# mhrice/RemFx

Measured on AMD Instinct MI355X. Metric: audio-seconds/sec fwd+bwd (whole job), higher is better.
Workload: dtype bf16 (fp32 accumulate); 1 GPU; Hybrid Demucs (cfg/model/demucs.yaml) train step, +exp=chorus_aug model=demucs; clips_per_gpu=64, global_batch=64, clip_samples=262144, parallelism=dp1, rccl_ranks=0, ranks=1, streams=4

## Files before the change

include/remfx_hip.h:

```cpp
#ifndef REMFX_HIP_H
#define REMFX_HIP_H

#include <stdint.h>

#ifdef __cplusplus
extern "C" {
#endif

#define RFX_ABI_VERSION 1

enum rfx_act {
  RFX_ACT_NONE = 0,
  RFX_ACT_RELU = 1,
  RFX_ACT_GELU = 2,
  RFX_ACT_TANH = 3,
  RFX_ACT_PRELU = 4,
  RFX_ACT_LEAKY = 5,
  RFX_ACT_SIGMOID = 6
};

typedef struct rfx_ktab_entry {
  int32_t off;
  int32_t da;
  int32_t db;
// ... 301 lines not shown
  int32_t N, IA, IB, OA, OB, SA;
  int32_t NTR, NCH, NTC, KS;
  int32_t da0, da_step;
  int32_t db0, db_step;
  int32_t wrapb;
  const void* apack;
  int32_t M, BM;
  int32_t mode;
  int32_t G, g_off, OAo, Co;
  const float* bias;
  const float* rowadd;
  rfx_cl_tensor out0, out1, aux0, res;
  void* cm_out;
  int64_t cm_ns, cm_cs, cm_as;
  int32_t cm_fold;
} rfx_cl_conv_desc;
int rfx_cl_conv(const rfx_cl_conv_desc* d, void* stream);
int rfx_cl_pack(const float* src, const int32_t* idx, int64_t n, void* dst, void* stream);
int rfx_cl_from_cm(const void* src, int32_t src_bf16, int64_t s_ns, int64_t s_cs, int64_t s_as, int32_t N, int32_t C, int32_t A,
                   int32_t B, const rfx_cl_tensor* dst, const rfx_cl_tensor* res, const rfx_cl_tensor* aux, int32_t mode, void* stream);
int rfx_cl_to_cm(const rfx_cl_tensor* src, int32_t N, int32_t C, int32_t A, int32_t B, void* dst, int32_t dst_bf16, int64_t d_ns,
                 int64_t d_cs, int64_t d_as, const void* aux16, void* stream);
int rfx_cl_im2col_s4(const float* src, int64_t s_ns, int64_t s_cs, int64_t s_as, int32_t N, int32_t Cs, int32_t IA, int32_t IB, int32_t OA,
                     int32_t OB, int32_t along_b, void* dst, void* stream);
int rfx_cl_im2col_fm(const float* src, const float* coef_a, const float* coef_b, int32_t N, int32_t F, int32_t bins, void* dst, void* stream);
int rfx_fm_cm_affine(const float* in, float* out, const float* coef_a, const float* coef_b, int32_t N, int32_t bins, int32_t F, int32_t to_fm,
                     void* stream);
int rfx_cl_dgelu(const void* g, const void* z, void* out, int64_t n, void* stream);
int rfx_cl_dglu(const void* g, const void* zab, void* out, int64_t npos, int32_t C, void* stream);

// ... 45 lines not shown
```

remfx_amd/_lib.py:

```python
import ctypes as C
import glob
import os
import subprocess

_HERE = os.path.dirname(os.path.abspath(__file__))
_ROOT = os.path.dirname(_HERE)
CSRC = os.path.join(_HERE, "csrc")
INCLUDE = os.path.join(_ROOT, "include")
LIBDIR = os.path.join(_HERE, "_C")
LIBPATH = os.environ.get("RFX_LIBPATH_DEV") or os.path.join(LIBDIR, "libremfx_hip.so")

HIPCC_FLAGS = ["--offload-arch=gfx950", "-O3", "-std=c++17", "-fPIC", "-ffp-contract=fast",
               "-I" + INCLUDE, "-I" + CSRC]


def sources():
    return sorted(glob.glob(os.path.join(CSRC, "*.hip")))


def _stale():
    if not os.path.exists(LIBPATH):
        return True
    t = os.path.getmtime(LIBPATH)
    deps = sources() + glob.glob(os.path.join(CSRC, "*.h")) + glob.glob(os.path.join(INCLUDE, "*.h"))
# ... 57 lines not shown
                                         "herm")] + \
               [(n, C.c_float) for n in ("scale", "eps", "alpha")] + [("accum", C.c_int32)]


class ClTensor(C.Structure):
    _fields_ = [("p", C.c_void_p), ("ns", C.c_int64), ("as_", C.c_int64), ("bs", C.c_int32), ("c0", C.c_int32)]


class ClConvDesc(C.Structure):
    _fields_ = [("inp", ClTensor)] + \
               [(n, C.c_int32) for n in ("N", "IA", "IB", "OA", "OB", "SA", "NTR", "NCH", "NTC", "KS", "da0", "da_step", "db0",
                                         "db_step", "wrapb")] + \
               [("apack", C.c_void_p)] + \
               [(n, C.c_int32) for n in ("M", "BM", "mode", "G", "g_off", "OAo", "Co")] + \
               [("bias", C.c_void_p), ("rowadd", C.c_void_p), ("out0", ClTensor), ("out1", ClTensor), ("aux0", ClTensor), ("res", ClTensor),
                ("cm_out", C.c_void_p), ("cm_ns", C.c_int64), ("cm_cs", C.c_int64), ("cm_as", C.c_int64), ("cm_fold", C.c_int32)]


class ClDconvDesc(C.Structure):
    _fields_ = [(n, C.c_void_p) for n in ("x", "gy", "y", "a", "hpre", "stats", "dz", "dh", "partial", "w1p", "w2p", "w2dp", "w1dp",
                                          "b1", "g1w", "g1b", "b2", "g2w", "g2b", "scale")] + \
               [(n, C.c_int32) for n in ("S", "C", "H", "dil", "grid", "x_or_gy_ok")] + [("eps", C.c_float), ("TPS", C.c_int32), ("tsum", C.c_void_p), ("sums", C.c_void_p), ("pg_dst", C.c_void_p * 5)]


class ClWgradDesc(C.Structure):
    _fields_ = [("p", ClTensor), ("q", ClTensor)] + \
               [(n, C.c_int32) for n in ("N", "OA", "IA", "B", "SA", "da0", "NTR", "NTC", "db0", "db_step", "M", "Cq", "CW", "RW", "WK",
                                         "S", "ahead", "bias", "PW")] + \
               [("ws", C.c_void_p)]


# ... 161 lines not shown
```

remfx_amd/clast.py:

```python
import ctypes as C
import os as _os

import numpy as np
import torch

from . import _lib, ops
from ._lib import ClConvDesc, ClTensor, ClWgradDesc, check

EPI = {"store": 0, "gelu": 1, "glu": 2, "dgelu": 3, "dglu": 4, "store_cm": 5}


def _stream():
    return C.c_void_p(ops.raw_stream())


def cl_tensor(t, c0=0):
    ct = ClTensor()
    if t is None:
        return ct
    if t.dtype != torch.bfloat16 or t.dim() != 4 or t.stride(3) != 1 or not t.is_cuda:
        raise ValueError(f"channels-last operand must be a 4-D bf16 GPU tensor with dense channels (got {t.dtype}, {tuple(t.shape)}, {t.stride()})")
    ct.p = t.data_ptr()
    ct.ns, ct.as_, ct.bs, ct.c0 = t.stride(0), t.stride(1), t.stride(2), c0
    return ct
# ... 104 lines not shown
        v = torch.from_numpy(form.idx).to(device)
        form._dev[key] = v
    return v


def pack(form, w):
    idx = _dev_index(form, w.device)
    wf = w if w.is_contiguous() else w.contiguous()
    out = torch.empty(idx.numel(), device=w.device, dtype=torch.bfloat16)
    check(_lib.lib().rfx_cl_pack(C.c_void_p(wf.data_ptr()), C.c_void_p(idx.data_ptr()), idx.numel(), C.c_void_p(out.data_ptr()),
                                 _stream()), "rfx_cl_pack")
    return out


def conv(form, apack, x, N, IA, IB, OA, mode, bias=None, out0=None, out1=None, aux0=None, res=None, OAo=0, x_c0=0, wrapb=False,
         rowadd=None, cm_out=None, cm_fold=False):
    d = ClConvDesc()
    d.inp = cl_tensor(x, x_c0)
    d.N, d.IA, d.IB, d.OA, d.OB, d.SA = N, IA, IB, OA, IB, form.SA
    d.NTR, d.NCH, d.NTC, d.KS = form.NTR, form.NCH, form.NTC, form.KS
    d.da0, d.da_step, d.db0, d.db_step = form.da0, form.da_step, form.db0, form.db_step
    d.wrapb = int(wrapb)
    d.apack = apack.data_ptr()
    d.M, d.BM, d.mode = form.M, form.BM, EPI[mode]
    d.G, d.g_off, d.OAo, d.Co = form.G, form.g_off, OAo, form.Co
    d.bias = bias.data_ptr() if bias is not None else None
    d.rowadd = rowadd.data_ptr() if rowadd is not None else None
    d.out0, d.out1, d.aux0, d.res = cl_tensor(out0), cl_tensor(out1), cl_tensor(aux0), cl_tensor(res)
    if cm_out is not None:
        if cm_out.dtype != torch.float32 or cm_out.stride(3) != 1:
            raise ValueError("store_cm: fp32 (N, C, rows, positions) with contiguous positions")
        d.cm_out, d.cm_ns, d.cm_cs, d.cm_as, d.cm_fold = cm_out.data_ptr(), cm_out.stride(0), cm_out.stride(1), cm_out.stride(2), int(cm_fold)
    check(_lib.lib().rfx_cl_conv(C.byref(d), _stream()), "rfx_cl_conv")


def form_conv_glu(Cout2, Cin, KA, KB):
    Ch = Cout2 // 2

    def widx(m, r, t, ch):
        oc = (m & 1) * Ch + (m >> 1)
        return ((oc * Cin + ch) * KA + r) * KB + t
    return ConvForm(Cout2, Cin, KA, KB, -(KA // 2), 1, -(KB // 2), 1, 1, widx)
# ... 284 lines not shown
```

remfx_amd/clchain.py:

```python
import ctypes as C

import torch

from . import _lib, clast, ops
from ._lib import check

_FORMS = {}
_BUILD = {
    "glu": clast.form_conv_glu, "dgrad": clast.form_conv_dgrad, "s4": clast.form_conv_s4, "s4d": clast.form_conv_s4_dgrad,
    "tr": clast.form_convtr_s4, "trd": clast.form_convtr_s4_dgrad, "w": clast.wform_conv, "ws4": clast.wform_conv_s4,
    "wtr": clast.wform_convtr_s4,
    "s4f": clast.form_conv_s4_fold, "s4fd": clast.form_conv_s4_fold_dgrad, "trf": clast.form_convtr_fold,
    "trfd": clast.form_convtr_fold_dgrad, "ws4f": clast.wform_conv_s4_fold, "wtrf": clast.wform_convtr_fold,
    "head": clast.form_head, "whead": clast.wform_head, "tail": clast.form_tail_tr, "taild": clast.form_tail_dgrad, "wtail": clast.wform_tail,
}


def _fold(t, k=4):
    N, A, L, Cc = t.shape
    return t.view(N, A, L // k, k * Cc)


def form(kind, *a):
    key = (kind,) + a
# ... 63 lines not shown
    return dw, db


def _scratch_bias(f, p):
    return torch.empty(f.M, device=p.device, dtype=torch.float32) if f.bias else None


def _as_ncab(x3, Bn, A):
    NA, Cc, T = x3.shape
    return x3.view(Bn, A, Cc, T).permute(0, 2, 1, 3)


class EncMidFn(torch.autograd.Function):

    @staticmethod
    def forward(ctx, d, rw_w, rw_b, cv_w, cv_b, emb_rows, Bn, y_cl, fold):
        d_is_cl = d.dim() == 4
        if d_is_cl:
            _, A, T, Cc = d.shape
            d_cl = d if d.is_contiguous() else d.contiguous()
        else:
            NA, Cc, T = d.shape
            A = NA // Bn
            d_cl = clast.from_cm(_as_ncab(d if d.is_contiguous() else d.contiguous(), Bn, A))
        C1 = cv_w.shape[0]
        A1, T1 = (A, T // 4) if fold else (A // 4, T)
        dev = d.device
        train = any(ctx.needs_input_grad)
        zab = clast.empty(Bn, A, T, 2 * Cc, dev) if train else None
        e = clast.empty(Bn, A, T, Cc, dev)
        fg = form("glu", 2 * Cc, Cc, 1, 1)
# ... 4 lines not shown
        if fold:
            fs = form("s4f", C1, Cc)
            clast.conv(fs, packed(fs, cv_w), _fold(e), Bn, 1, T1, 1, "gelu", bias=cv_b, out0=z1, out1=y1)
        else:
            fs = form("s4", C1, Cc)
            clast.conv(fs, packed(fs, cv_w), e, Bn, A, T, A1, "gelu", bias=cv_b, out0=z1, out1=y1)
        if y_cl:
            y_out = y1
        else:
            y_out = torch.empty((Bn * A1, C1, T1), device=dev, dtype=torch.float32)
            clast.to_cm(y1, out=_as_ncab(y_out, Bn, A1))
        if train:
            ctx.save_for_backward(d_cl, zab, e, z1, rw_w, cv_w)
            ctx.refs = (rw_b, cv_b)
            ctx.geom = (Bn, A, T, Cc, C1, A1, T1, emb_rows is not None, d_is_cl, y_cl, fold)
        return e, y_out

    @staticmethod
    def backward(ctx, g_e, g_y):
        d_cl, zab, e, z1, rw_w, cv_w = ctx.saved_tensors
        rw_b, cv_b = ctx.refs
        Bn, A, T, Cc, C1, A1, T1, has_emb, d_is_cl, y_cl, fold = ctx.geom
        dev = d_cl.device
        if y_cl:
            dz1 = clast.dgelu(g_y if g_y.is_contiguous() else g_y.contiguous(), z1)
        else:
            dz1 = clast.empty(Bn, A1, T1, C1, dev)
            clast.from_cm(_as_ncab(g_y if g_y.is_contiguous() else g_y.contiguous(), Bn, A1), out=dz1, aux=z1, mode="dgelu")
        g_e = (g_e if g_e.is_contiguous() else g_e.contiguous()) if g_e is not None else None
        if fold:
            dcw, dcb = _wgrad(form("ws4f", C1, Cc), dz1, _fold(e), Bn, 1, 1, T1, cv_w, cv_b)
            fd = form("s4fd", C1, Cc)
            v = clast.empty(Bn, A, T, Cc, dev)
            clast.conv(fd, packed(fd, cv_w), dz1, Bn, 1, T1, 1, "store", out0=_fold(v), res=_fold(g_e) if g_e is not None else None)
            dzab = clast.dglu(v, zab)
        else:
            dcw, dcb = _wgrad(form("ws4", C1, Cc), dz1, e, Bn, A1, A, T, cv_w, cv_b)
            fd = form("s4d", C1, Cc)
            dzab = clast.empty(Bn, A, T, 2 * Cc, dev)
            v = clast.empty(Bn, A, T, Cc, dev) if has_emb else None
            clast.conv(fd, packed(fd, cv_w), dz1, Bn, A1, T, A1 + 1, "dglu", out0=dzab, out1=v, aux0=zab, res=g_e, OAo=A)
        demb = None
        if has_emb:
            demb = torch.empty((A, Cc), device=dev, dtype=torch.float32)
            rowsum(v, A, Cc, demb)
        drw, drb = _wgrad(form("w", 2 * Cc, Cc, 1, 1), dzab, d_cl, Bn, A, A, T, rw_w, rw_b)
        fr = form("dgrad", 2 * Cc, Cc, 1, 1)
        dd_cl = clast.empty(Bn, A, T, Cc, dev)
        clast.conv(fr, packed(fr, rw_w), dzab, Bn, A, T, A, "store", out0=dd_cl)
        if d_is_cl:
            dd = dd_cl
        else:
            dd = torch.empty((Bn * A, Cc, T), device=dev, dtype=torch.float32)
            clast.to_cm(dd_cl, out=_as_ncab(dd, Bn, A))
        return dd, drw, drb, dcw, dcb, demb, None, None, None


class EncTailFn(torch.autograd.Function):

    @staticmethod
    def forward(ctx, d, rw_w, rw_b, Bn):
        d_is_cl = d.dim() == 4
        if d_is_cl:
            _, A, T, Cc = d.shape
            d_cl = d if d.is_contiguous() else d.contiguous()
        else:
            NA, Cc, T = d.shape
            A = NA // Bn
            d_cl = clast.from_cm(_as_ncab(d if d.is_contiguous() else d.contiguous(), Bn, A))
        dev = d.device
# ... 163 lines not shown
class HeadGeluFn(torch.autograd.Function):

    @staticmethod
    def forward(ctx, z):
        ctx.save_for_backward(z)
        return clast.from_cm(z, mode="gelu")

    @staticmethod
    def backward(ctx, g):
        (z,) = ctx.saved_tensors
        gz = torch.empty_like(z)
        clast.to_cm(g if g.is_contiguous() else g.contiguous(), out=gz, aux16=z)
        return gz


def head_gelu(z):
    if z.dtype != torch.bfloat16 or not z.is_contiguous():
        raise ValueError("head_gelu: contiguous bf16 (N, C, A, T)")
    return HeadGeluFn.apply(z)


def _w4(w):
    return w if w.dim() == 4 else w.unsqueeze(2)


def enc_mid(d, rewrite, conv_next, emb_rows, Bn, y_cl=False, fold=False):
    return EncMidFn.apply(d, _w4(rewrite.weight), rewrite.bias, _w4(conv_next.weight), conv_next.bias, emb_rows, Bn, y_cl, fold)


def enc_tail(d, rewrite, Bn):
    return EncTailFn.apply(d, _w4(rewrite.weight), rewrite.bias, Bn)


def freq_decoder(x, skips, layers, fold=False, tail=False):
    params = []
    for m in layers[:-1]:
        params += [_w4(m.rewrite.weight), m.rewrite.bias, _w4(m.conv_tr.weight), m.conv_tr.bias]
    params += [_w4(layers[-1].rewrite.weight), layers[-1].rewrite.bias]
    if tail:
        params += [_w4(layers[-1].conv_tr.weight), layers[-1].conv_tr.bias]
    return FreqDecoderFn.apply(x, len(skips), fold, tail, *skips, *params)


class HeadConvFn(torch.autograd.Function):

    @staticmethod
    def forward(ctx, x, w, b, along_b, coef=None):
        if coef is not None:
            Bn, T, IA, Cs = x.shape
            A = IA // 4
            x16 = clast.im2col_fm(x, coef[0], coef[1])
        else:
            Bn, Cs, IA, T = x.shape
            A, T = (IA, T // 4) if along_b else (IA // 4, T)
            x16 = clast.im2col_s4(x, A, T, along_b)
        Cc = w.shape[0]
        dev = x.device
        train = any(ctx.needs_input_grad[1:3])
        f = form("head", Cc, Cs)
        z = clast.empty(Bn, A, T, Cc, dev) if train else None
        y = clast.empty(Bn, A, T, Cc, dev)
        clast.conv(f, packed(f, w), x16, Bn, A, T, A, "gelu", bias=b, out0=z, out1=y)
        if train:
            ctx.save_for_backward(x16, z, w)
            ctx.refs = (b,)
        return y

    @staticmethod
    def backward(ctx, g):
        x16, z, w = ctx.saved_tensors
        (b,) = ctx.refs
        Bn, A, T, Cc = z.shape
        dz = clast.dgelu(g if g.is_contiguous() else g.contiguous(), z)
        dw, db = _wgrad(form("whead", Cc, w.shape[1]), dz, x16, Bn, A, A, T, w, b)
        return None, dw, db, None, None


def head_conv(x, conv, along_b=False):
    return HeadConvFn.apply(x, _w4(conv.weight), conv.bias, along_b)


def head_conv_fm(spec_fm, a, b, conv):
    return HeadConvFn.apply(spec_fm, _w4(conv.weight), conv.bias, False, (a, b))
```

remfx_amd/cldconv.py:

```python
import ctypes as C

import numpy as np
import torch

from . import _lib, clast, clchain, ops
from ._lib import ClDconvDesc, check

T = 256
import os as _os
GRID = 256
GRID_FWD = int(_os.environ.get("RFX_CLD_GRID_FWD", "256"))


class _Idx:

    def __init__(self, idx):
        self.idx = np.ascontiguousarray(idx.reshape(-1).astype(np.int32))
        self._dev = {}


_TABLES = {}


def tables(Cc, H):
# ... 64 lines not shown

def _p(t):
    return t.data_ptr() if t is not None else None


def _desc(Cc, H, dil, eps, S, b1, g1w, g1b, b2, g2w, g2b, scale):
    d = ClDconvDesc()
    d.S, d.C, d.H, d.dil, d.grid, d.eps = S, Cc, H, dil, GRID, eps
    d.b1, d.g1w, d.g1b, d.b2, d.g2w, d.g2b, d.scale = _p(b1), _p(g1w), _p(g1b), _p(b2), _p(g2w), _p(g2b), _p(scale)
    return d


class ClDconvLayerFn(torch.autograd.Function):

    @staticmethod
    def forward(ctx, x, w1, b1, g1w, g1b, w2, b2, g2w, g2b, scale, dil, eps):
        Bn, A, Tt, Cc = x.shape
        H = w1.shape[0]
        if Tt % T or not x.is_contiguous() or x.dtype != torch.bfloat16:
            raise ValueError("ClDconvLayerFn: dense (N, A, 256 k, C) bf16 input")
        tb = tables(Cc, H)
        TPS = Tt // T
        HP, S, dev = tb["HP"], Bn * A * TPS, x.device
        train = any(ctx.needs_input_grad)
        y = torch.empty_like(x)
        d = _desc(Cc, H, dil, eps, S, b1, g1w, g1b, b2, g2w, g2b, scale)
        d.TPS = TPS
        d.grid = GRID_FWD
        d.x, d.y = x.data_ptr(), y.data_ptr()
        d.w1p = clchain.packed(tb["w1p"], w1).data_ptr()
        d.w2p = clchain.packed(tb["w2p"], w2).data_ptr()
        a = hpre = stats = part = None
        if train or TPS > 1:
            stats = torch.empty((Bn * A, 4), device=dev, dtype=torch.float32)
            d.stats = stats.data_ptr()
        if TPS > 1:
            part = torch.empty((S, 2), device=dev, dtype=torch.float32)
            d.partial = part.data_ptr()
        if train:
            a = torch.empty((Bn, A, Tt, HP), device=dev, dtype=torch.bfloat16)
            hpre = torch.empty_like(a)
            d.a, d.hpre = a.data_ptr(), hpre.data_ptr()
        check(_lib.lib().rfx_cl_dconv_fwd(C.byref(d), C.c_void_p(ops.raw_stream())), "rfx_cl_dconv_fwd")
        if train:
            ctx.save_for_backward(x, a, hpre, stats, w1, b1, g1w, g1b, w2, b2, g2w, g2b, scale)
            ctx.cfg = (dil, eps)
        return y

    @staticmethod
    def backward(ctx, gy):
        x, a, hpre, stats, w1, b1, g1w, g1b, w2, b2, g2w, g2b, scale = ctx.saved_tensors
        dil, eps = ctx.cfg
        Bn, A, Tt, Cc = x.shape
        H = w1.shape[0]
        tb = tables(Cc, H)
        TPS = Tt // T
        HP, S, dev = tb["HP"], Bn * A * TPS, x.device
        passes = TPS > 1 or Cc != 48
        if not gy.is_contiguous():
            gy = gy.contiguous()
        dx = torch.empty_like(x)
        dz = torch.empty((Bn, A, Tt, 2 * Cc), device=dev, dtype=torch.bfloat16)
        dh = torch.empty((Bn, A, Tt, HP), device=dev, dtype=torch.bfloat16)
        npg = 5 * Cc + 2 * H
        partial = torch.empty((min(GRID, S), npg), device=dev, dtype=torch.float32)
        sink = ops.SINK
# ... 10 lines not shown
            tsum = torch.empty((S, 2), device=dev, dtype=torch.float32)
            sums = torch.empty((Bn * A, 4), device=dev, dtype=torch.float32)
            d.tsum, d.sums = tsum.data_ptr(), sums.data_ptr()
        else:
            d.w1dp = clchain.packed(tb["w1dp"], w1).data_ptr()
        if direct:
            for q, t in enumerate(tgt):
                d.pg_dst[q] = t[1].data_ptr()
        check(_lib.lib().rfx_cl_dconv_bwd(C.byref(d), C.c_void_p(pg.data_ptr() if pg is not None else None), C.c_void_p(ops.raw_stream())),
              "rfx_cl_dconv_bwd")
        if direct:
            for t in tgt:
                sink.wrote(t[0])
        if passes:
            fx = _dx_form(Cc, H, dil)
            clast.conv(fx, clchain.packed(fx, w1), dh, Bn, A, Tt, A, "store", out0=dx, res=gy)
        f1, f2 = _wforms(Cc, H, dil)
        dw2, db2 = clchain._wgrad(f2, dz, a, Bn, A, A, Tt, w2, b2)
        dw1, db1 = clchain._wgrad(f1, dh, x, Bn, A, A, Tt, w1, b1)
        if direct:
            dscale = dg2w = dg2b = dg1w = dg1b = None
        else:
            dscale, dg2w, dg2b = pg[:Cc], pg[Cc:3 * Cc], pg[3 * Cc:5 * Cc]
            dg1w, dg1b = pg[5 * Cc:5 * Cc + H], pg[5 * Cc + H:]
        return dx, dw1, db1, dg1w, dg1b, dw2, db2, dg2w, dg2b, dscale, None, None


def dconv_layer(x, conv1, gn1, conv2, gn2, scale, dil):
    return ClDconvLayerFn.apply(x, conv1.weight, conv1.bias, gn1.weight, gn1.bias, conv2.weight, conv2.bias, gn2.weight, gn2.bias,
                                scale, int(dil), float(gn1.eps))
```

remfx_amd/csrc/cl_conv.h:

```cpp
#pragma once
#include "cl_common.h"

#ifndef RFX_CLC_DBG_BUILD
#define RFX_CLC_DBG_BUILD 0
#endif

struct ClConvK {
  rfx_cl_conv_desc d;
  int32_t ptiles, chunk, MG, tpr;
  uint32_t in_bytes;
};

template <int RW, int NT, int WM, int NTC, int KS, int DA, int DB, bool HALO>
struct ClConvCfg {
  static constexpr int WN = 8 / WM, BM = 32 * RW * WM, MT = RW * WM;
  static constexpr int A_KB = NTC * KS * MT;
  static constexpr int PA = (A_KB + 3) / 4;
  static constexpr int SLOTS = HALO ? 272 : 256, CORE0 = HALO ? 16 : 0, PLANE = SLOTS * 32;
  static constexpr int PB = KS * (HALO ? 3 : 2);
  static constexpr int A_UNIT = A_KB * 1024, B_UNIT = KS * PLANE;
  static constexpr int RING = DA * A_UNIT + DB * B_UNIT;
  static constexpr int EPI_RS = 64 * RW + 8, EPI_RSY = 32 * RW + 8;
  static constexpr int EPI_WAVE = 32 * EPI_RS + 32 * EPI_RSY;
  static constexpr int BIAS_OFF = (RING > 8 * EPI_WAVE ? RING : 8 * EPI_WAVE);
// ... 355 lines not shown
        cl_unpack8(raw, v);
        if (mode == RFX_CL_GELU || mode == RFX_CL_DGELU) {
          if (has0) cl_bst(rs0, off0, raw);
          float w[8];
          if (has_aux) cl_unpack8(cl_bld(rsx, (uint32_t)(((int64_t)orow * d.aux0.as + (int64_t)bp * d.aux0.bs + ch) * 2)), w);
          float o[8];
          if (mode == RFX_CL_GELU) {
#pragma unroll
            for (int e = 0; e < 8; ++e) o[e] = rfx_gelu(v[e]) + (has_aux ? w[e] : 0.f);
          } else {
#pragma unroll
            for (int e = 0; e < 8; ++e) o[e] = v[e] * rfx_gelu_grad(w[e]);
          }
          cl_bst(rs1, (uint32_t)(((int64_t)orow * d.out1.as + (int64_t)bp * d.out1.bs + ch) * 2), cl_pack8(o));
        } else {
          const uint32_t ax = (uint32_t)(((int64_t)orow * d.aux0.as + (int64_t)bp * d.aux0.bs + ch) * 2);
          const int half = d.aux0.bs >> 1;
          float a[8], b[8], ga[8], gb[8];
          if (has1) cl_bst(rs1, (uint32_t)(((int64_t)orow * d.out1.as + (int64_t)bp * d.out1.bs + ch) * 2), raw);
          cl_unpack8(cl_bld(rsx, ax), a);
          cl_unpack8(cl_bld(rsx, ax + half * 2), b);
#pragma unroll
          for (int e = 0; e < 8; ++e) {
            const float s = rfx_sigmoid(b[e]);
            ga[e] = v[e] * s;
            gb[e] = v[e] * a[e] * s * (1.f - s);
          }
          cl_bst(rs0, off0, cl_pack8(ga));
          cl_bst(rs0, off0 + half * 2, cl_pack8(gb));
        }
      }
    }
    __builtin_amdgcn_wave_barrier();
    CL_LGKM0();
  }
}

template <int MODE, int RW, int NT, int WM, int NTC, int KS, int DA, int DB, bool HALO>
static int cl_conv_launch(const ClConvK& k, dim3 grid, hipStream_t s) {
  using Cfg = ClConvCfg<RW, NT, WM, NTC, KS, DA, DB, HALO>;
  static bool attr_done = false;
  if (!attr_done) {
    if (hipFuncSetAttribute(reinterpret_cast<const void*>(&cl_conv_kernel<MODE, RW, NT, WM, NTC, KS, DA, DB, HALO>),
                            hipFuncAttributeMaxDynamicSharedMemorySize, Cfg::LDS) != hipSuccess)
// ... 41 lines not shown
```

remfx_amd/csrc/cl_conv.hip:

```cpp
#include "cl_conv.h"

static bool cl_fits32(const rfx_cl_tensor& t, int rows, int IB) {
  if (!t.p) return true;
  return ((int64_t)rows * t.as + (int64_t)IB * t.bs) * 2 < 0x7fffffffLL && t.bs % 8 == 0 && t.c0 % 8 == 0;
}

extern "C" int rfx_cl_conv(const rfx_cl_conv_desc* dp, void* stream) {
  if (!dp || !dp->in.p || !dp->apack) return -1;
  const rfx_cl_conv_desc& d = *dp;
  if (d.N <= 0 || d.OA <= 0 || d.OB <= 0 || d.OB % 256 || d.OB != d.IB || d.M <= 0 || d.NTR <= 0 || d.NTR > 16 || d.NCH <= 0) return -1;
  if (d.in.bs % 8 || d.in.c0 % 8 || (d.NCH * 16 * d.KS + d.in.c0) > d.in.bs) return -1;
  const bool cm = d.mode == RFX_CL_STORE_CM;
  if (d.G < 1 || d.G > 4 || (d.G > 1 && ((!cm && d.Co % 8) || d.Co * d.G != d.M))) return -1;
  if (d.mode < 0 || d.mode > RFX_CL_STORE_CM) return -1;
  if (cm && (!d.cm_out || d.Co <= 0 || d.M % d.Co || d.BM != 32)) return -1;
  if (d.mode == RFX_CL_GLU && (d.M % 16 || !d.out1.p || d.G != 1)) return -1;
  if ((d.mode == RFX_CL_STORE || d.mode == RFX_CL_DGLU) && !d.out0.p) return -1;
  if ((d.mode == RFX_CL_GELU || d.mode == RFX_CL_DGELU) && !d.out1.p) return -1;
  if ((d.mode == RFX_CL_DGELU || d.mode == RFX_CL_DGLU) && !d.aux0.p) return -1;
  if (d.M % 8 && !cm) return -1;
  const int orows = d.G > 1 ? d.OAo : d.OA;
  if (!cl_fits32(d.out0, orows, d.IB) || !cl_fits32(d.out1, orows, d.IB) || !cl_fits32(d.aux0, orows, d.IB) || !cl_fits32(d.res, orows, d.IB))
    return -1;
  const int64_t ext = ((int64_t)(d.IA - 1) * d.in.as + (int64_t)d.IB * d.in.bs - d.in.c0) * 2;
  if (ext <= 0 || ext >= 0x7fffffffLL) return -1;
  ClConvK k;
  k.d = d;
  k.tpr = d.OB / 256;
  k.ptiles = d.N * d.OA * k.tpr;
  k.chunk = (k.ptiles + 7) / 8;
  k.MG = (d.M + d.BM - 1) / d.BM;
  k.in_bytes = (uint32_t)ext;

  const dim3 grid((unsigned)(8 * k.chunk * k.MG));
// ... 28 lines not shown
```

remfx_amd/hdemucs.py:

```python
import math
import os

import torch
import torch.nn as nn
import torch.nn.functional as F

from . import clchain, cldconv, lstm, nnops, ops, stft

CL_TRUNK = os.environ.get("RFX_CL_TRUNK", "1") != "0"
CL_TIME = os.environ.get("RFX_CL_TIME", "1") != "0"
CL_ENDS = os.environ.get("RFX_CL_ENDS", "1") != "0"
FM_ENDS = os.environ.get("RFX_FM_ENDS", "1") != "0"
TWO_STREAMS = os.environ.get("RFX_TWO_STREAMS", "1") != "0"
_TIME_STREAMS = {}


def _data_parallel():
    if not (torch.distributed.is_available() and torch.distributed.is_initialized() and torch.distributed.get_world_size() > 1):
        return False
    return torch.is_grad_enabled() and ops.SINK is None


def _dev_env(name, default):
    v = os.environ.get(name)
    if v is None or v == default:
        return default
    if os.environ.get("RFX_DEV") != "1":
        import warnings
        warnings.warn(f"{name}={v} ignored: development switch, set RFX_DEV=1 to honour it")
        return default
    import warnings
    warnings.warn(f"RFX_DEV=1: development switch {name}={v} is ACTIVE and changes what the network computes or how it is ordered")
    return v


_XSUB = int(_dev_env("RFX_XSYNC_SUB", "0"))
_CUR = [None, None]
_XIDX = int(_dev_env("RFX_XSYNC_IDX", "-1"))
_XSYNC = int(_dev_env("RFX_XSYNC", "0"))


def _time_stream(device):
    idx = device.index if device.index is not None else torch.cuda.current_device()
    st = _TIME_STREAMS.get(idx)
    if st is None:
        st = torch.cuda.Stream(device=idx, priority=-1)
        _TIME_STREAMS[idx] = st
    return st
# ... 103 lines not shown
                mods.insert(3, _LocalState(hidden, heads=heads, ndecay=ndecay))
            if lstm:
                mods.insert(3, _BLSTM(hidden, layers=2, skip=True))
            self.layers.append(nn.Sequential(*mods))
            self.spec.append((dil, dil * (kernel_size // 2), lstm, attn))

    def cl_ok(self, positions=256):
        for seq, (dil, pad, lstm, attn) in zip(self.layers, self.spec):
            m = list(seq)
            if lstm or attn or m[0].kernel_size[0] != 3 or dil not in (1, 2) or m[1].eps != m[4].eps or m[1].num_groups != 1:
                return False
            if not cldconv.supported(m[0].in_channels, m[0].out_channels, True, positions):
                return False
        return True

    def forward_cl(self, x):
        for seq, (dil, pad, lstm, attn) in zip(self.layers, self.spec):
            m = list(seq)
            x = cldconv.dconv_layer(x, m[0], m[1], m[3], m[4], m[6].scale, dil)
        return x

    def forward(self, x):
        if _DBG_SKIP and self.layers[0][0].in_channels in _DBG_SKIP:
            return x
        for seq, (dil, pad, lstm, attn) in zip(self.layers, self.spec):
            mods = list(seq)
            if (not lstm and not attn and mods[1].eps == mods[4].eps and mods[1].num_groups == 1 and
                    nnops.dconv_layer_fused_ok(x, mods[0].out_channels, mods[0].kernel_size[0], dil,
                                               torch.is_grad_enabled() and (x.requires_grad or mods[0].weight.requires_grad))):
                x = nnops.dconv_layer(x, mods[0], mods[1], mods[3], mods[4], mods[6].scale, dil)
                continue
            st = _stat_buf(x) if DCONV_EPI_STATS else None
            y, x = ops.conv1d_fork(x, mods[0].weight, mods[0].bias, 1, pad, dil, stat_sums=st, out_bf16=True)
            if _DCONV_DBG is not None:
# ... 278 lines not shown

    def _cl_layers_time(self, length, device, Lc):
        if not CL_TIME or Lc == 0 or len(self.time_encoder) <= Lc or length % (4 ** Lc * 256):
            return 0
        for i in range(Lc):
            enc, dec = self.time_encoder[i], self.time_decoder[len(self.time_decoder) - 1 - i]
            ok = (not enc.freq and not enc.empty and enc.context == 0 and enc.kernel_size == 8 and enc.stride == 4 and enc.pad == 2
                  and not isinstance(enc.norm1, nn.GroupNorm) and not isinstance(enc.norm2, nn.GroupNorm)
                  and enc.conv.out_channels % 16 == 0
                  and not dec.freq and not dec.empty and dec.context == 1 and dec.kernel_size == 8 and dec.stride == 4 and dec.pad == 2
                  and not isinstance(dec.norm1, nn.GroupNorm) and not isinstance(dec.norm2, nn.GroupNorm))
            if not ok:
                return 0
        return Lc

    def _time_encoder_step(self, idx, Lt, B, saved_t, lengths_t, xt, samp_t, len_t):
        inject = None
        tenc = self.time_encoder[idx]
        if idx < Lt:
            lengths_t.append(len_t)
            len_t = len_t // 4
            tdcl = CL_DCONV and CL_TIME_DCONV and tenc.dconv.cl_ok(len_t)
            if idx == 0:
                if tdcl and CL_ENDS and xt.shape[1] == 1 and not xt.requires_grad:
                    samp_t = clchain.head_conv(xt.unsqueeze(2), tenc.conv, along_b=True)
                else:
                    samp_t, tdcl = tenc.head_t(xt), False
            dt_ = tenc.dconv.forward_cl(samp_t) if tdcl else tenc.dconv(samp_t)
            if _XSUB and _CUR[0] is not None and _XIDX in (-1, idx):
                if _XSUB & 1:
                    _CUR[0].wait_stream(_CUR[1])
                if _XSUB & 2:
                    _CUR[1].wait_stream(_CUR[0])
            if idx < Lt - 1:
                nxt_t = CL_DCONV and CL_TIME_DCONV and self.time_encoder[idx + 1].dconv.cl_ok(len_t // 4)
                et, samp_t = clchain.enc_mid(dt_, tenc.rewrite, self.time_encoder[idx + 1].conv, None, B, y_cl=nxt_t, fold=True)
            else:
                et, xt = clchain.enc_tail(dt_, tenc.rewrite, B)
                xt = xt.squeeze(2)
            saved_t.append(et)
        else:
            lengths_t.append(xt.shape[-1])
            if saved_t and saved_t[-1] is xt:
                xt, alias = tenc(xt, fork=True)
                if alias is not None:
                    saved_t[-1] = alias
            else:
                xt = tenc(xt)
            if not tenc.empty:
                saved_t.append(xt)
            else:
                inject = xt
        return xt, samp_t, len_t, inject

    def forward(self, input):
        if input.ndim != 3 or input.shape[1] != self.audio_channels:
            raise ValueError(f"expected (batch, {self.audio_channels}, frames), got {tuple(input.shape)}")
        ops._req(input, "input")
        B, Cin, length = input.shape
        hl = self.hop_length
        le = math.ceil(length / hl)
        pad = hl // 2 * 3
        if input.requires_grad:
            raise NotImplementedError("HDemucs: gradient w.r.t. the input waveform is not on the reference's path")
        saved, saved_t, lengths, lengths_t = [], [], [], []
        Lc = self._cl_layers(le, input.device)
        Lt = self._cl_layers_time(length, input.device, Lc)
        samp = samp_t = None
        len_t = length
        import contextlib
        two = TWO_STREAMS and input.is_cuda and Lt > 0 and not _data_parallel()
        xt, meant, stdt = nnops.row_standardize(input, 1e-5)
        if two:
            main_s, time_s = torch.cuda.current_stream(), _time_stream(input.device)
            time_s.wait_stream(main_s)
            xt.record_stream(time_s)
        tctx = (lambda: torch.cuda.stream(time_s)) if two else contextlib.nullcontext
        _CUR[0], _CUR[1] = (main_s, time_s) if two else (None, None)
        Fq = self.nfft // 2
        fm = (FM_ENDS and Lc > 0 and CL_ENDS and CL_DCONV and Cin == 1 and Fq % 4 == 0 and len(self.sources) == 1
              and self.freq_encoder[0].dconv.cl_ok())
        if fm:
            spec_fm = stft.stft(input.reshape(B * Cin, length), self.nfft, hl, mode="complex_fm", normalized=True,
                                bins=Fq, frame0=2, frames_out=le, extra_pad=(pad, pad + le * hl - length)).detach()
            mean, std, coef_a, coef_b = nnops.row_moments(spec_fm, 1e-5)
            x = None
        else:
            cac = stft.stft(input.reshape(B * Cin, length), self.nfft, hl, mode="cac", normalized=True,
                            bins=self.nfft // 2, frame0=2, frames_out=le, extra_pad=(pad, pad + le * hl - length))
            x = cac.view(B, Cin, 2, Fq, le).reshape(B, Cin * 2, Fq, le)
            x, mean, std = nnops.row_standardize(x.detach(), 1e-5)
        for idx, encode in enumerate(self.freq_encoder):
            lengths.append(le if x is None else x.shape[-1])
            inject = None
            if idx < len(self.time_encoder):
                if two and (_XSYNC & 2) and _XIDX in (-1, idx):
                    time_s.wait_stream(main_s)
                with tctx():
                    xt, samp_t, len_t, inject = self._time_encoder_step(idx, Lt, B, saved_t, lengths_t, xt, samp_t, len_t)
                if two and (_XSYNC & 1) and _XIDX in (-1, idx):
                    main_s.wait_stream(time_s)
                if two and inject is not None:
                    main_s.wait_stream(time_s)
                    inject.record_stream(main_s)
            if idx < Lc:
                dcl = CL_DCONV and encode.dconv.cl_ok()
                if idx == 0:
                    samp = clchain.head_conv_fm(spec_fm, coef_a, coef_b, encode.conv) if fm else encode.head(x, cl=dcl, ends=CL_ENDS)
                d = encode.dconv.forward_cl(samp) if dcl else encode.dconv(samp)
                if getattr(self, "_dbg", None) is not None and not dcl:
                    csn = lambda t: t.float().abs().reshape(B, -1).sum(1) if t.is_contiguous() else t.float().abs().contiguous().reshape(B, -1).sum(1)
                    self._dbg.setdefault("samp", {})[idx] = csn(samp)
                    self._dbg.setdefault("d", {})[idx] = csn(d)
                if idx < Lc - 1:
                    emb_rows = self.freq_emb.table() * self.freq_emb_scale if (idx == 0 and self.freq_emb is not None) else None
                    nxt = CL_DCONV and self.freq_encoder[idx + 1].dconv.cl_ok()
                    e, samp = clchain.enc_mid(d, encode.rewrite, self.freq_encoder[idx + 1].conv, emb_rows, B, y_cl=nxt)
                else:
                    e, x = clchain.enc_tail(d, encode.rewrite, B)
                saved.append(e)
                continue
            if saved and saved[-1] is x:
                x, alias = encode(x, inject, fork=True)
                if alias is not None:
                    saved[-1] = alias
            else:
                x = encode(x, inject)
            if idx == 0 and self.freq_emb is not None:
                emb = self.freq_emb.table().t()[None, :, :, None]
                x = nnops.add(x, emb, self.freq_emb_scale)
            saved.append(x)
        x = ops.zeros(x.shape, x.device)
# ... 81 lines not shown
```

remfx_amd/ops.py:

```python
import ctypes as C

import numpy as np
import torch

from . import _lib, convplan
from ._lib import Epilogue, GemmDesc, check

import os as _os
PREC_NAMES = {"f32": 0, "bf16x3": 1, "bf16": 2}
GEMM_PREC = PREC_NAMES[_os.environ.get("RFX_GEMM_PREC", "f32")]


BF16_STORE = True


def bf16_storage():
    return GEMM_PREC == 2 and BF16_STORE


def set_gemm_precision(name):
    global GEMM_PREC
    GEMM_PREC = PREC_NAMES[name]


def gemm_precision():
# ... 809 lines not shown
```

Measured before the change: 3728 audio-seconds/sec.

## Fuse GELU/GLU backward epilogues into channels-last conv backward passes

Adds a pre-activation handoff (PreAct) so the first DConv layer's dx conv applies gelu'(z) of the previous encoder's output in its epilogue, letting the upstream conv backward skip a separate dgelu pass. In the folded time-encoder path, the dglu is also fused into the transposed conv epilogue via a new glu_g grouping parameter, removing an intermediate tensor and a separate elementwise kernel. This saves memory traffic from standalone elementwise backward kernels but couples autograd nodes across modules through shared state, and adds a runtime check that raises if the handoff is not consumed.

Result: no change. 3723 audio-seconds/sec (-0.1%).

```diff
diff --git a/include/remfx_hip.h b/include/remfx_hip.h
--- a/include/remfx_hip.h
+++ b/include/remfx_hip.h
@@ -339,6 +339,7 @@
   void* cm_out;
   int64_t cm_ns, cm_cs, cm_as;
   int32_t cm_fold;
+  int32_t glu_g;
 } rfx_cl_conv_desc;
 int rfx_cl_conv(const rfx_cl_conv_desc* d, void* stream);
 int rfx_cl_pack(const float* src, const int32_t* idx, int64_t n, void* dst, void* stream);
diff --git a/remfx_amd/_lib.py b/remfx_amd/_lib.py
--- a/remfx_amd/_lib.py
+++ b/remfx_amd/_lib.py
@@ -95,7 +95,7 @@
                [("apack", C.c_void_p)] + \
                [(n, C.c_int32) for n in ("M", "BM", "mode", "G", "g_off", "OAo", "Co")] + \
                [("bias", C.c_void_p), ("rowadd", C.c_void_p), ("out0", ClTensor), ("out1", ClTensor), ("aux0", ClTensor), ("res", ClTensor),
-                ("cm_out", C.c_void_p), ("cm_ns", C.c_int64), ("cm_cs", C.c_int64), ("cm_as", C.c_int64), ("cm_fold", C.c_int32)]
+                ("cm_out", C.c_void_p), ("cm_ns", C.c_int64), ("cm_cs", C.c_int64), ("cm_as", C.c_int64), ("cm_fold", C.c_int32), ("glu_g", C.c_int32)]
 
 
 class ClDconvDesc(C.Structure):
diff --git a/remfx_amd/clast.py b/remfx_amd/clast.py
--- a/remfx_amd/clast.py
+++ b/remfx_amd/clast.py
@@ -142,7 +142,7 @@
 
 
 def conv(form, apack, x, N, IA, IB, OA, mode, bias=None, out0=None, out1=None, aux0=None, res=None, OAo=0, x_c0=0, wrapb=False,
-         rowadd=None, cm_out=None, cm_fold=False):
+         rowadd=None, cm_out=None, cm_fold=False, glu_g=0):
     d = ClConvDesc()
     d.inp = cl_tensor(x, x_c0)
     d.N, d.IA, d.IB, d.OA, d.OB, d.SA = N, IA, IB, OA, IB, form.SA
@@ -154,6 +154,7 @@
     d.G, d.g_off, d.OAo, d.Co = form.G, form.g_off, OAo, form.Co
     d.bias = bias.data_ptr() if bias is not None else None
     d.rowadd = rowadd.data_ptr() if rowadd is not None else None
+    d.glu_g = glu_g
     d.out0, d.out1, d.aux0, d.res = cl_tensor(out0), cl_tensor(out1), cl_tensor(aux0), cl_tensor(res)
     if cm_out is not None:
         if cm_out.dtype != torch.float32 or cm_out.stride(3) != 1:
diff --git a/remfx_amd/clchain.py b/remfx_amd/clchain.py
--- a/remfx_amd/clchain.py
+++ b/remfx_amd/clchain.py
@@ -4,6 +4,20 @@
 
 from . import _lib, clast, ops
 from ._lib import check
+
+TAIL_FUSION = ops.dev_env("RFX_CL_TAIL_FUSION", "1") != "0"
+
+
+class PreAct:
+
+    def __init__(self):
+        self.z = None
+        self.taken = False
+
+    def take(self):
+        self.taken = self.z is not None
+        return self.z
+
 
 _FORMS = {}
 _BUILD = {
@@ -101,7 +115,7 @@
 class EncMidFn(torch.autograd.Function):
 
     @staticmethod
-    def forward(ctx, d, rw_w, rw_b, cv_w, cv_b, emb_rows, Bn, y_cl, fold):
+    def forward(ctx, d, rw_w, rw_b, cv_w, cv_b, emb_rows, Bn, y_cl, fold, preact=None):
         d_is_cl = d.dim() == 4
         if d_is_cl:
             _, A, T, Cc = d.shape
@@ -136,6 +150,9 @@
             ctx.save_for_backward(d_cl, zab, e, z1, rw_w, cv_w)
             ctx.refs = (rw_b, cv_b)
             ctx.geom = (Bn, A, T, Cc, C1, A1, T1, emb_rows is not None, d_is_cl, y_cl, fold)
+            ctx.preact = preact if y_cl else None
+            if ctx.preact is not None:
+                preact.z = z1
         return e, y_out
 
     @staticmethod
@@ -145,7 +162,8 @@
         Bn, A, T, Cc, C1, A1, T1, has_emb, d_is_cl, y_cl, fold = ctx.geom
         dev = d_cl.device
         if y_cl:
-            dz1 = clast.dgelu(g_y if g_y.is_contiguous() else g_y.contiguous(), z1)
+            g_y = g_y if g_y.is_contiguous() else g_y.contiguous()
+            dz1 = g_y if _premultiplied(ctx.preact) else clast.dgelu(g_y, z1)
         else:
             dz1 = clast.empty(Bn, A1, T1, C1, dev)
             clast.from_cm(_as_ncab(g_y if g_y.is_contiguous() else g_y.contiguous(), Bn, A1), out=dz1, aux=z1, mode="dgelu")
@@ -153,9 +171,14 @@
         if fold:
             dcw, dcb = _wgrad(form("ws4f", C1, Cc), dz1, _fold(e), Bn, 1, 1, T1, cv_w, cv_b)
             fd = form("s4fd", C1, Cc)
-            v = clast.empty(Bn, A, T, Cc, dev)
-            clast.conv(fd, packed(fd, cv_w), dz1, Bn, 1, T1, 1, "store", out0=_fold(v), res=_fold(g_e) if g_e is not None else None)
-            dzab = clast.dglu(v, zab)
+            res = _fold(g_e) if g_e is not None else None
+            if TAIL_FUSION:
+                dzab = clast.empty(Bn, A, T, 2 * Cc, dev)
+                clast.conv(fd, packed(fd, cv_w), dz1, Bn, 1, T1, 1, "dglu", out0=_fold(dzab), aux0=_fold(zab), res=res, glu_g=Cc)
+            else:
+                v = clast.empty(Bn, A, T, Cc, dev)
+                clast.conv(fd, packed(fd, cv_w), dz1, Bn, 1, T1, 1, "store", out0=_fold(v), res=res)
+                dzab = clast.dglu(v, zab)
         else:
             dcw, dcb = _wgrad(form("ws4", C1, Cc), dz1, e, Bn, A1, A, T, cv_w, cv_b)
             fd = form("s4d", C1, Cc)
@@ -175,7 +198,7 @@
         else:
             dd = torch.empty((Bn * A, Cc, T), device=dev, dtype=torch.float32)
             clast.to_cm(dd_cl, out=_as_ncab(dd, Bn, A))
-        return dd, drw, drb, dcw, dcb, demb, None, None, None
+        return dd, drw, drb, dcw, dcb, demb, None, None, None, None
 
 
 class EncTailFn(torch.autograd.Function):
@@ -369,6 +392,14 @@
         return gz
 
 
+def _premultiplied(preact):
+    if preact is None:
+        return False
+    if not preact.taken:
+        raise RuntimeError("a pre-activation was handed over (PreAct) but no DConv branch took it: its gradient lacks gelu'(z)")
+    return True
+
+
 def head_gelu(z):
     if z.dtype != torch.bfloat16 or not z.is_contiguous():
         raise ValueError("head_gelu: contiguous bf16 (N, C, A, T)")
@@ -379,8 +410,8 @@
     return w if w.dim() == 4 else w.unsqueeze(2)
 
 
-def enc_mid(d, rewrite, conv_next, emb_rows, Bn, y_cl=False, fold=False):
-    return EncMidFn.apply(d, _w4(rewrite.weight), rewrite.bias, _w4(conv_next.weight), conv_next.bias, emb_rows, Bn, y_cl, fold)
+def enc_mid(d, rewrite, conv_next, emb_rows, Bn, y_cl=False, fold=False, preact=None):
+    return EncMidFn.apply(d, _w4(rewrite.weight), rewrite.bias, _w4(conv_next.weight), conv_next.bias, emb_rows, Bn, y_cl, fold, preact)
 
 
 def enc_tail(d, rewrite, Bn):
@@ -400,7 +431,7 @@
 class HeadConvFn(torch.autograd.Function):
 
     @staticmethod
-    def forward(ctx, x, w, b, along_b, coef=None):
+    def forward(ctx, x, w, b, along_b, coef=None, preact=None):
         if coef is not None:
             Bn, T, IA, Cs = x.shape
             A = IA // 4
@@ -419,6 +450,9 @@
         if train:
             ctx.save_for_backward(x16, z, w)
             ctx.refs = (b,)
+            ctx.preact = preact
+            if preact is not None:
+                preact.z = z
         return y
 
     @staticmethod
@@ -426,13 +460,14 @@
         x16, z, w = ctx.saved_tensors
         (b,) = ctx.refs
         Bn, A, T, Cc = z.shape
-        dz = clast.dgelu(g if g.is_contiguous() else g.contiguous(), z)
+        g = g if g.is_contiguous() else g.contiguous()
+        dz = g if _premultiplied(ctx.preact) else clast.dgelu(g, z)
         dw, db = _wgrad(form("whead", Cc, w.shape[1]), dz, x16, Bn, A, A, T, w, b)
-        return None, dw, db, None, None
-
-
-def head_conv(x, conv, along_b=False):
-    return HeadConvFn.apply(x, _w4(conv.weight), conv.bias, along_b)
+        return None, dw, db, None, None, None
+
+
+def head_conv(x, conv, along_b=False, preact=None):
+    return HeadConvFn.apply(x, _w4(conv.weight), conv.bias, along_b, None, preact)
 
 
 def head_conv_fm(spec_fm, a, b, conv):
diff --git a/remfx_amd/cldconv.py b/remfx_amd/cldconv.py
--- a/remfx_amd/cldconv.py
+++ b/remfx_amd/cldconv.py
@@ -102,7 +102,7 @@
 class ClDconvLayerFn(torch.autograd.Function):
 
     @staticmethod
-    def forward(ctx, x, w1, b1, g1w, g1b, w2, b2, g2w, g2b, scale, dil, eps):
+    def forward(ctx, x, w1, b1, g1w, g1b, w2, b2, g2w, g2b, scale, dil, eps, zprev=None):
         Bn, A, Tt, Cc = x.shape
         H = w1.shape[0]
         if Tt % T or not x.is_contiguous() or x.dtype != torch.bfloat16:
@@ -131,13 +131,15 @@
             d.a, d.hpre = a.data_ptr(), hpre.data_ptr()
         check(_lib.lib().rfx_cl_dconv_fwd(C.byref(d), C.c_void_p(ops.raw_stream())), "rfx_cl_dconv_fwd")
         if train:
-            ctx.save_for_backward(x, a, hpre, stats, w1, b1, g1w, g1b, w2, b2, g2w, g2b, scale)
+            if zprev is not None and (zprev.shape != x.shape or zprev.dtype != torch.bfloat16 or not zprev.is_contiguous()):
+                raise ValueError("ClDconvLayerFn: zprev must be a dense bf16 tensor of x's shape")
+            ctx.save_for_backward(x, a, hpre, stats, w1, b1, g1w, g1b, w2, b2, g2w, g2b, scale, zprev)
             ctx.cfg = (dil, eps)
         return y
 
     @staticmethod
     def backward(ctx, gy):
-        x, a, hpre, stats, w1, b1, g1w, g1b, w2, b2, g2w, g2b, scale = ctx.saved_tensors
+        x, a, hpre, stats, w1, b1, g1w, g1b, w2, b2, g2w, g2b, scale, zprev = ctx.saved_tensors
         dil, eps = ctx.cfg
         Bn, A, Tt, Cc = x.shape
         H = w1.shape[0]
@@ -178,7 +180,14 @@
                 sink.wrote(t[0])
         if passes:
             fx = _dx_form(Cc, H, dil)
-            clast.conv(fx, clchain.packed(fx, w1), dh, Bn, A, Tt, A, "store", out0=dx, res=gy)
+            if zprev is not None and clchain.TAIL_FUSION:
+                clast.conv(fx, clchain.packed(fx, w1), dh, Bn, A, Tt, A, "dgelu", out1=dx, aux0=zprev, res=gy)
+            else:
+                clast.conv(fx, clchain.packed(fx, w1), dh, Bn, A, Tt, A, "store", out0=dx, res=gy)
+                if zprev is not None:
+                    dx = clast.dgelu(dx, zprev)
+        elif zprev is not None:
+            dx = clast.dgelu(dx, zprev)
         f1, f2 = _wforms(Cc, H, dil)
         dw2, db2 = clchain._wgrad(f2, dz, a, Bn, A, A, Tt, w2, b2)
         dw1, db1 = clchain._wgrad(f1, dh, x, Bn, A, A, Tt, w1, b1)
@@ -187,9 +196,9 @@
         else:
             dscale, dg2w, dg2b = pg[:Cc], pg[Cc:3 * Cc], pg[3 * Cc:5 * Cc]
             dg1w, dg1b = pg[5 * Cc:5 * Cc + H], pg[5 * Cc + H:]
-        return dx, dw1, db1, dg1w, dg1b, dw2, db2, dg2w, dg2b, dscale, None, None
-
-
-def dconv_layer(x, conv1, gn1, conv2, gn2, scale, dil):
+        return dx, dw1, db1, dg1w, dg1b, dw2, db2, dg2w, dg2b, dscale, None, None, None
+
+
+def dconv_layer(x, conv1, gn1, conv2, gn2, scale, dil, zprev=None):
     return ClDconvLayerFn.apply(x, conv1.weight, conv1.bias, gn1.weight, gn1.bias, conv2.weight, conv2.bias, gn2.weight, gn2.bias,
-                                scale, int(dil), float(gn1.eps))
+                                scale, int(dil), float(gn1.eps), zprev)
diff --git a/remfx_amd/csrc/cl_conv.h b/remfx_amd/csrc/cl_conv.h
--- a/remfx_amd/csrc/cl_conv.h
+++ b/remfx_amd/csrc/cl_conv.h
@@ -393,8 +393,10 @@
           }
           cl_bst(rs1, (uint32_t)(((int64_t)orow * d.out1.as + (int64_t)bp * d.out1.bs + ch) * 2), cl_pack8(o));
         } else {
-          const uint32_t ax = (uint32_t)(((int64_t)orow * d.aux0.as + (int64_t)bp * d.aux0.bs + ch) * 2);
-          const int half = d.aux0.bs >> 1;
+          const int half = d.glu_g > 0 ? d.glu_g : d.aux0.bs >> 1;
+          const int shift = d.glu_g > 0 ? (ch / d.glu_g) * d.glu_g : 0;
+          const uint32_t ax = (uint32_t)(((int64_t)orow * d.aux0.as + (int64_t)bp * d.aux0.bs + ch + shift) * 2);
+          const uint32_t og = off0 + (uint32_t)(shift * 2);
           float a[8], b[8], ga[8], gb[8];
           if (has1) cl_bst(rs1, (uint32_t)(((int64_t)orow * d.out1.as + (int64_t)bp * d.out1.bs + ch) * 2), raw);
           cl_unpack8(cl_bld(rsx, ax), a);
@@ -405,8 +407,8 @@
             ga[e] = v[e] * s;
             gb[e] = v[e] * a[e] * s * (1.f - s);
           }
-          cl_bst(rs0, off0, cl_pack8(ga));
-          cl_bst(rs0, off0 + half * 2, cl_pack8(gb));
+          cl_bst(rs0, og, cl_pack8(ga));
+          cl_bst(rs0, og + half * 2, cl_pack8(gb));
         }
       }
     }
diff --git a/remfx_amd/csrc/cl_conv.hip b/remfx_amd/csrc/cl_conv.hip
--- a/remfx_amd/csrc/cl_conv.hip
+++ b/remfx_amd/csrc/cl_conv.hip
@@ -18,6 +18,8 @@
   if ((d.mode == RFX_CL_STORE || d.mode == RFX_CL_DGLU) && !d.out0.p) return -1;
   if ((d.mode == RFX_CL_GELU || d.mode == RFX_CL_DGELU) && !d.out1.p) return -1;
   if ((d.mode == RFX_CL_DGELU || d.mode == RFX_CL_DGLU) && !d.aux0.p) return -1;
+  if (d.glu_g < 0 || (d.glu_g > 0 && (d.mode != RFX_CL_DGLU || d.G != 1 || d.glu_g % 8 || d.M % d.glu_g))) return -1;
+  if (d.glu_g > 0 && (2 * d.M + d.out0.c0 > d.out0.bs || 2 * d.M + d.aux0.c0 > d.aux0.bs)) return -1;
   if (d.M % 8 && !cm) return -1;
   const int orows = d.G > 1 ? d.OAo : d.OA;
   if (!cl_fits32(d.out0, orows, d.IB) || !cl_fits32(d.out1, orows, d.IB) || !cl_fits32(d.aux0, orows, d.IB) || !cl_fits32(d.res, orows, d.IB))
diff --git a/remfx_amd/hdemucs.py b/remfx_amd/hdemucs.py
--- a/remfx_amd/hdemucs.py
+++ b/remfx_amd/hdemucs.py
@@ -21,17 +21,7 @@
     return torch.is_grad_enabled() and ops.SINK is None
 
 
-def _dev_env(name, default):
-    v = os.environ.get(name)
-    if v is None or v == default:
-        return default
-    if os.environ.get("RFX_DEV") != "1":
-        import warnings
-        warnings.warn(f"{name}={v} ignored: development switch, set RFX_DEV=1 to honour it")
-        return default
-    import warnings
-    warnings.warn(f"RFX_DEV=1: development switch {name}={v} is ACTIVE and changes what the network computes or how it is ordered")
-    return v
+_dev_env = ops.dev_env
 
 
 _XSUB = int(_dev_env("RFX_XSYNC_SUB", "0"))
@@ -165,10 +155,12 @@
                 return False
         return True
 
-    def forward_cl(self, x):
+    def forward_cl(self, x, preact=None):
+        zprev = preact.take() if preact is not None else None
         for seq, (dil, pad, lstm, attn) in zip(self.layers, self.spec):
             m = list(seq)
-            x = cldconv.dconv_layer(x, m[0], m[1], m[3], m[4], m[6].scale, dil)
+            x = cldconv.dconv_layer(x, m[0], m[1], m[3], m[4], m[6].scale, dil, zprev=zprev)
+            zprev = None
         return x
 
     def forward(self, x):
@@ -477,7 +469,7 @@
                 return 0
         return Lc
 
-    def _time_encoder_step(self, idx, Lt, B, saved_t, lengths_t, xt, samp_t, len_t):
+    def _time_encoder_step(self, idx, Lt, B, saved_t, lengths_t, xt, samp_t, pre_t, len_t):
         inject = None
         tenc = self.time_encoder[idx]
         if idx < Lt:
@@ -486,10 +478,12 @@
             tdcl = CL_DCONV and CL_TIME_DCONV and tenc.dconv.cl_ok(len_t)
             if idx == 0:
                 if tdcl and CL_ENDS and xt.shape[1] == 1 and not xt.requires_grad:
-                    samp_t = clchain.head_conv(xt.unsqueeze(2), tenc.conv, along_b=True)
+                    pre_t = clchain.PreAct()
+                    samp_t = clchain.head_conv(xt.unsqueeze(2), tenc.conv, along_b=True, preact=pre_t)
                 else:
                     samp_t, tdcl = tenc.head_t(xt), False
-            dt_ = tenc.dconv.forward_cl(samp_t) if tdcl else tenc.dconv(samp_t)
+            dt_ = tenc.dconv.forward_cl(samp_t, pre_t) if tdcl else tenc.dconv(samp_t)
+            pre_t = None
             if _XSUB and _CUR[0] is not None and _XIDX in (-1, idx):
                 if _XSUB & 1:
                     _CUR[0].wait_stream(_CUR[1])
@@ -497,7 +491,8 @@
                     _CUR[1].wait_stream(_CUR[0])
             if idx < Lt - 1:
                 nxt_t = CL_DCONV and CL_TIME_DCONV and self.time_encoder[idx + 1].dconv.cl_ok(len_t // 4)
-                et, samp_t = clchain.enc_mid(dt_, tenc.rewrite, self.time_encoder[idx + 1].conv, None, B, y_cl=nxt_t, fold=True)
+                pre_t = clchain.PreAct() if nxt_t else None
+                et, samp_t = clchain.enc_mid(dt_, tenc.rewrite, self.time_encoder[idx + 1].conv, None, B, y_cl=nxt_t, fold=True, preact=pre_t)
             else:
                 et, xt = clchain.enc_tail(dt_, tenc.rewrite, B)
                 xt = xt.squeeze(2)
@@ -514,7 +509,7 @@
                 saved_t.append(xt)
             else:
                 inject = xt
-        return xt, samp_t, len_t, inject
+        return xt, samp_t, pre_t, len_t, inject
 
     def forward(self, input):
         if input.ndim != 3 or input.shape[1] != self.audio_channels:
@@ -529,7 +524,7 @@
         saved, saved_t, lengths, lengths_t = [], [], [], []
         Lc = self._cl_layers(le, input.device)
         Lt = self._cl_layers_time(length, input.device, Lc)
-        samp = samp_t = None
+        samp = samp_t = pre = pre_t = None
         len_t = length
         import contextlib
         two = TWO_STREAMS and input.is_cuda and Lt > 0 and not _data_parallel()
@@ -560,7 +555,7 @@
                 if two and (_XSYNC & 2) and _XIDX in (-1, idx):
                     time_s.wait_stream(main_s)
                 with tctx():
-                    xt, samp_t, len_t, inject = self._time_encoder_step(idx, Lt, B, saved_t, lengths_t, xt, samp_t, len_t)
+                    xt, samp_t, pre_t, len_t, inject = self._time_encoder_step(idx, Lt, B, saved_t, lengths_t, xt, samp_t, pre_t, len_t)
                 if two and (_XSYNC & 1) and _XIDX in (-1, idx):
                     main_s.wait_stream(time_s)
                 if two and inject is not None:
@@ -570,7 +565,8 @@
                 dcl = CL_DCONV and encode.dconv.cl_ok()
                 if idx == 0:
                     samp = clchain.head_conv_fm(spec_fm, coef_a, coef_b, encode.conv) if fm else encode.head(x, cl=dcl, ends=CL_ENDS)
-                d = encode.dconv.forward_cl(samp) if dcl else encode.dconv(samp)
+                d = encode.dconv.forward_cl(samp, pre) if dcl else encode.dconv(samp)
+                pre = None
                 if getattr(self, "_dbg", None) is not None and not dcl:
                     csn = lambda t: t.float().abs().reshape(B, -1).sum(1) if t.is_contiguous() else t.float().abs().contiguous().reshape(B, -1).sum(1)
                     self._dbg.setdefault("samp", {})[idx] = csn(samp)
@@ -578,7 +574,8 @@
                 if idx < Lc - 1:
                     emb_rows = self.freq_emb.table() * self.freq_emb_scale if (idx == 0 and self.freq_emb is not None) else None
                     nxt = CL_DCONV and self.freq_encoder[idx + 1].dconv.cl_ok()
-                    e, samp = clchain.enc_mid(d, encode.rewrite, self.freq_encoder[idx + 1].conv, emb_rows, B, y_cl=nxt)
+                    pre = clchain.PreAct() if nxt else None
+                    e, samp = clchain.enc_mid(d, encode.rewrite, self.freq_encoder[idx + 1].conv, emb_rows, B, y_cl=nxt, preact=pre)
                 else:
                     e, x = clchain.enc_tail(d, encode.rewrite, B)
                 saved.append(e)
diff --git a/remfx_amd/ops.py b/remfx_amd/ops.py
--- a/remfx_amd/ops.py
+++ b/remfx_amd/ops.py
@@ -9,6 +9,18 @@
 import os as _os
 PREC_NAMES = {"f32": 0, "bf16x3": 1, "bf16": 2}
 GEMM_PREC = PREC_NAMES[_os.environ.get("RFX_GEMM_PREC", "f32")]
+
+
+def dev_env(name, default):
+    v = _os.environ.get(name)
+    if v is None or v == default:
+        return default
+    import warnings
+    if _os.environ.get("RFX_DEV") != "1":
+        warnings.warn(f"{name}={v} ignored: development switch, set RFX_DEV=1 to honour it")
+        return default
+    warnings.warn(f"RFX_DEV=1: development switch {name}={v} is ACTIVE and changes what the network computes or how it is ordered")
+    return v
 
 
 BF16_STORE = True
```
